# TUI-NICR/nicr-multitask-scene-analysis

Hardware: AMD Instinct MI355X
Metric: Mpix/s panoptic merge+metrics, 640x480xB (higher is better)
Workload: dtype f32; 1 GPU; configs[1]: center-NMS + offset grouping + panoptic merge + mIoU/PQ accumulators (configs[3]); batch_per_gpu=32, global_batch=32, classes=40, height=480, width=640, centers_per_image=24, batches_in_flight=2, parallelism=dp1 (images sharded, accumulators all-reduced once per run, timed)

## Files before the change

nicr_mt_scene_analysis_amd/csrc/panoptic.hip:

```cpp
#include <stdlib.h>
#include <type_traits>

#include "nmsa_common.hpp"
#include "argmax_state.hpp"

namespace nmsa {

constexpr int FUSED_THREADS = 256;
constexpr int FUSED_VOTE_SLOTS = 256;
constexpr int PX_PER_THREAD = 4;
constexpr int PX_PER_ITER = FUSED_THREADS * PX_PER_THREAD;

typedef float f32x4_t __attribute__((ext_vector_type(4)));
typedef unsigned short u16x4_t __attribute__((ext_vector_type(4)));

template <int DTYPE, bool VEC, bool NT = false>
__device__ __forceinline__ float4 load_px4(const void* base, size_t elem_off, int nvalid)
{
    float4 r = make_float4(0.f, 0.f, 0.f, 0.f);
    if (DTYPE == NMSA_F32) {
        const float* p = (const float*)base + elem_off;
        if (VEC && NT) {
            const f32x4_t v = __builtin_nontemporal_load((const f32x4_t*)p);
            return make_float4(v.x, v.y, v.z, v.w);
        }
        if (VEC) return *(const float4*)p;
        if (nvalid > 0) r.x = p[0];
        if (nvalid > 1) r.y = p[1];
        if (nvalid > 2) r.z = p[2];
        if (nvalid > 3) r.w = p[3];
        return r;
    } else {
        const uint16_t* p = (const uint16_t*)base + elem_off;
        uint16_t h[4] = {0, 0, 0, 0};
        if (VEC && NT) {
            const u16x4_t u = __builtin_nontemporal_load((const u16x4_t*)p);
            h[0] = u.x; h[1] = u.y; h[2] = u.z; h[3] = u.w;
        } else if (VEC) {
            const ushort4 u = *(const ushort4*)p;
            h[0] = u.x; h[1] = u.y; h[2] = u.z; h[3] = u.w;
        } else {
            for (int j = 0; j < 4; ++j) if (j < nvalid) h[j] = p[j];
        }
        if (DTYPE == NMSA_BF16) {
            r.x = bf16_to_f32(h[0]); r.y = bf16_to_f32(h[1]);
            r.z = bf16_to_f32(h[2]); r.w = bf16_to_f32(h[3]);
        } else {
            r.x = f16_to_f32(h[0]); r.y = f16_to_f32(h[1]);
            r.z = f16_to_f32(h[2]); r.w = f16_to_f32(h[3]);
        }
        return r;
    }
}

template <int DTYPE>
__device__ __noinline__ int column_class(const void* logits, size_t col0, int P, int C, float m)
{
    auto ld = [&](int c) -> float {
        if (DTYPE == NMSA_F32) return ((const float*)logits)[col0 + (size_t)c * P];
        const uint16_t h = ((const uint16_t*)logits)[col0 + (size_t)c * P];
        return (DTYPE == NMSA_BF16) ? bf16_to_f32(h) : f16_to_f32(h);
    };
    bool nan_or_pinf = false, any_finite = false;
    int first = C, am = C;
    int c = 0;
    for (; c + 4 <= C; c += 4) {
        float v[4];
#pragma unroll
        for (int u = 0; u < 4; ++u) v[u] = ld(c + u);
#pragma unroll
        for (int u = 0; u < 4; ++u) {
            nan_or_pinf |= (v[u] != v[u]) || (v[u] == INFINITY);
            any_finite |= fabsf(v[u]) < INFINITY;
            if (first == C && __fsub_rn(v[u], m) >= TIE_CANDIDATE_GAP) first = c + u;
            if (am == C && v[u] == m) am = c + u;
        }
    }
    for (; c < C; ++c) {
        const float v = ld(c);
        nan_or_pinf |= (v != v) || (v == INFINITY);
        any_finite |= fabsf(v) < INFINITY;
        if (first == C && __fsub_rn(v, m) >= TIE_CANDIDATE_GAP) first = c;
        if (am == C && v == m) am = c;
    }
    if (nan_or_pinf || !any_finite || am == C) return 0;
    if (first >= am) return am;
    return class_by_probability(ld, C, m, am, first, nullptr);
}

template <int DTYPE>
__device__ __noinline__ float2 column_exact(const void* logits, size_t col0, int P, int C)
{
    auto ld = [&](int c) -> float {
        if (DTYPE == NMSA_F32) return ((const float*)logits)[col0 + (size_t)c * P];
        const uint16_t h = ((const uint16_t*)logits)[col0 + (size_t)c * P];
        return (DTYPE == NMSA_BF16) ? bf16_to_f32(h) : f16_to_f32(h);
    };
    bool nan_or_pinf = false, any_finite = false;
    float m = -INFINITY;
    int am = 0;
    for (int c = 0; c < C; ++c) {
        const float v = ld(c);
        if (v != v || v == INFINITY) nan_or_pinf = true;
        if (fabsf(v) < INFINITY) any_finite = true;
        if (v > m) { m = v; am = c; }
    }
    if (nan_or_pinf || !any_finite) return make_float2(__int_as_float(0x7fc00000), __int_as_float(0));
    float se = 0.f;
    int first = am;
    for (int c = 0; c < C; ++c) {
        const float v = ld(c);
        se += (v == -INFINITY) ? 0.f : __expf(v - m);
        if (c < first && __fsub_rn(v, m) >= TIE_CANDIDATE_GAP) first = c;
    }
    if (first >= am) return make_float2(1.0f / se, __int_as_float(am));
    float pm;
    const int cls = class_by_probability(ld, C, m, am, first, &pm);
    return make_float2(pm, __int_as_float(cls));
}

template <bool WITH_SCORE>
__device__ __forceinline__ void argmax_quad(ArgmaxState& st, const float4& a, const float4& b,
                                            const float4& c, const float4& d, int c0,
                                            int nclasses = 4)
{
    if (WITH_SCORE) {
        const float p0[4] = {a.x, b.x, c.x, d.x}, p1[4] = {a.y, b.y, c.y, d.y};
        const float p2[4] = {a.z, b.z, c.z, d.z}, p3[4] = {a.w, b.w, c.w, d.w};
        argmax_group4_score(st, 0, p0, c0);
        argmax_group4_score(st, 1, p1, c0);
        argmax_group4_score(st, 2, p2, c0);
        argmax_group4_score(st, 3, p3, c0);
    } else {
        const float4 q[4] = {a, b, c, d};
#pragma unroll
        for (int u = 0; u < 4; ++u) {
            if (u >= nclasses) break;
            argmax_step<false>(st, 0, q[u].x, c0 + u);
            argmax_step<false>(st, 1, q[u].y, c0 + u);
            argmax_step<false>(st, 2, q[u].z, c0 + u);
            argmax_step<false>(st, 3, q[u].w, c0 + u);
        }
    }
}

__device__ __forceinline__ float sqdist(float cy, float cx, float ly, float lx)
{
    const float dy = __fsub_rn(cy, ly);
    const float dx = __fsub_rn(cx, lx);
    return __fmaf_rn(dx, dx, __fmul_rn(dy, dy));
}

__device__ __forceinline__ float sqrt_tie_upper(float d)
{
    if (!(d < INFINITY)) return d;
    const float dn = __uint_as_float(__float_as_uint(d) + 1u);
    const double m = 0.5 * ((double)d + (double)dn);
    const double m2 = m * m;
    float u = (float)m2;
    if ((double)u >= m2) u = __uint_as_float(__float_as_uint(u) - 1u);
    return u;
}

__device__ __forceinline__ float wave_all_min(float v)
{
#pragma unroll
    for (int o = 32; o > 0; o >>= 1) v = fminf(v, __shfl_xor(v, o));
    return v;
}

struct LdsCenters {
    const float2* cen;
    __device__ __forceinline__ float2 at(int i) const { return cen[i]; }
    __device__ __forceinline__ float2 of_lane(int n) const { return cen[min(lane_id(), n - 1)]; }
};
struct LaneCenters {
    float cy, cx;
    __device__ __forceinline__ float2 at(int i) const
    {
        return make_float2(__int_as_float(__builtin_amdgcn_readlane(__float_as_int(cy), i)),
                           __int_as_float(__builtin_amdgcn_readlane(__float_as_int(cx), i)));
    }
    __device__ __forceinline__ float2 of_lane(int) const { return make_float2(cy, cx); }
};

template <typename Centers>
__device__ __forceinline__ uint64_t wave_candidate_centers(const Centers& cen, int n,
                                                           const float ly[4], const float lx[4],
                                                           const bool act[4])
{
    float lo_y = INFINITY, lo_x = INFINITY, nhi_y = INFINITY, nhi_x = INFINITY;
    bool finite = true;
#pragma unroll
    for (int j = 0; j < 4; ++j) {
        if (act[j]) {
            finite = finite && (fabsf(ly[j]) < INFINITY) && (fabsf(lx[j]) < INFINITY);
            lo_y = fminf(lo_y, ly[j]);  nhi_y = fminf(nhi_y, -ly[j]);
            lo_x = fminf(lo_x, lx[j]);  nhi_x = fminf(nhi_x, -lx[j]);
        }
    }
    const uint64_t all = (n >= 64) ? ~0ull : ((1ull << n) - 1ull);
    if (__any(!finite)) return all;
    lo_y = wave_all_min(lo_y);  nhi_y = wave_all_min(nhi_y);
    lo_x = wave_all_min(lo_x);  nhi_x = wave_all_min(nhi_x);
    if (!(lo_y < INFINITY)) return 0ull;
    const float hi_y = -nhi_y, hi_x = -nhi_x;
    const int lane = lane_id();
    const float2 c = cen.of_lane(n);
    const float a0 = c.x - lo_y, a1 = hi_y - c.x;
    const float b0 = c.y - lo_x, b1 = hi_x - c.y;
    const float near_y = fmaxf(0.f, fmaxf(-a0, -a1)), near_x = fmaxf(0.f, fmaxf(-b0, -b1));
    const float far_y = fmaxf(fabsf(a0), fabsf(a1)), far_x = fmaxf(fabsf(b0), fabsf(b1));
    const float lo = near_y * near_y + near_x * near_x;
    const float hi = (lane < n) ? far_y * far_y + far_x * far_x : INFINITY;
    const float U = wave_all_min(hi);
    return __ballot(lane < n && lo <= U * 1.00001f) & all;
}

template <bool CULL = true, typename Centers = LdsCenters>
__device__ __forceinline__ void group4(const Centers& cen, int n,
                                       const float ly[4], const float lx[4],
                                       const bool act[4], int use_thr, float thr,
                                       uint32_t id[4])
{
    float smin[4], prev[4];
    int imin[4];
    const bool cull = CULL && n <= 64;
    uint64_t m = cull ? wave_candidate_centers(cen, n, ly, lx, act) : 0ull;
    int first = 0;
    if (cull) {
        if (m == 0ull) {
#pragma unroll
            for (int j = 0; j < 4; ++j) id[j] = 0u;
            return;
        }
        first = __ffsll((unsigned long long)m) - 1;
        m &= m - 1;
    }
    {
        const float2 c0 = cen.at(first);
#pragma unroll
        for (int j = 0; j < 4; ++j) {
            smin[j] = sqdist(c0.x, c0.y, ly[j], lx[j]);
            prev[j] = INFINITY;
            imin[j] = first;
        }
    }
    auto visit = [&](const int i) {
        const float2 c = cen.at(i);
#pragma unroll
        for (int j = 0; j < 4; ++j) {
            const float s = sqdist(c.x, c.y, ly[j], lx[j]);
            const bool upd = s < smin[j];
            prev[j] = upd ? smin[j] : prev[j];
            imin[j] = upd ? i : imin[j];
            smin[j] = upd ? s : smin[j];
        }
    };
    if (cull) {
        while (m) {
            const int i = __ffsll((unsigned long long)m) - 1;
            m &= m - 1;
            visit(i);
        }
    } else {
        for (int i = 1; i < n; ++i) visit(i);
    }
    bool maybe_tie = false;
#pragma unroll
    for (int j = 0; j < 4; ++j)
        maybe_tie = maybe_tie || (act[j] && !(prev[j] > fmaf(smin[j], 4.8e-7f, smin[j])));
    int best[4] = {imin[0], imin[1], imin[2], imin[3]};
    if (__any(maybe_tie)) {
        float U[4];
#pragma unroll
        for (int j = 0; j < 4; ++j) U[j] = sqrt_tie_upper(sqrtf(smin[j]));
        for (int i = n - 1; i >= 0; --i) {
            const float2 c = cen.at(i);
#pragma unroll
            for (int j = 0; j < 4; ++j)
                if (sqdist(c.x, c.y, ly[j], lx[j]) <= U[j]) best[j] = i;
        }
#pragma unroll
        for (int j = 0; j < 4; ++j) best[j] = (smin[j] != smin[j]) ? 0 : best[j];
    }
#pragma unroll
    for (int j = 0; j < 4; ++j) {
        uint32_t v = (uint32_t)(best[j] + 1) & 0xFFu;
        if (use_thr && sqrtf(smin[j]) > thr) v = 0;
        id[j] = act[j] ? v : 0u;
    }
}

template <int DTYPE, bool VEC, bool WITH_SCORE, int UNROLL = 8, bool NT = true,
          bool EARLY_OFFSETS = false, bool TILED = false, int TILE_LOG2W = 6>
__global__ __launch_bounds__(FUSED_THREADS) __attribute__((amdgpu_waves_per_eu(5, WITH_SCORE ? 8 : 5))) void k_panoptic_fused(
    const void* __restrict__ logits, const float* __restrict__ offset,
    const int32_t* __restrict__ centers_yx, const int32_t* __restrict__ n_centers,
    const uint8_t* __restrict__ is_thing,
    int C, int H, int W, int max_centers, int iters,
    float scale_y, float scale_x, int use_thr, float thr,
    uint8_t* __restrict__ sem_u8, uint8_t* __restrict__ inst, uint8_t* __restrict__ fg_out,
    float* __restrict__ score, uint32_t* __restrict__ votes, int ablate)
{
    extern __shared__ __align__(16) unsigned char smem[];
    float2* cen = (float2*)smem;
    int* vote_key = (int*)(cen + max_centers);
    uint32_t* vote_cnt = (uint32_t*)(vote_key + FUSED_VOTE_SLOTS);
    const int NC = C + 1;

    const int b = blockIdx.y;
    const int P = H * W;
    const int n = min(n_centers[b], max_centers);

    static_assert(FUSED_THREADS == 256, "one LUT entry per thread");
    static_assert(FUSED_VOTE_SLOTS == FUSED_THREADS, "one vote slot per thread");
    vote_key[threadIdx.x] = -1;
    vote_cnt[threadIdx.x] = 0;
    const bool lane_centers = n <= 64 && H <= 65535 && W <= 65535;
    uint32_t lane_cyx, thing_b = 0u;
    {
        const int2 c2 = *(const int2*)(centers_yx +
            ((size_t)b * max_centers + min(lane_id(), max_centers - 1)) * 2);
        lane_cyx = ((uint32_t)c2.x << 16) | ((uint32_t)c2.y & 0xFFFFu);
#pragma unroll
        for (int k = 0; k < 4; ++k)
            if (k * 64 < C)
                thing_b |= (is_thing[min(k * 64 + lane_id(), C - 1)] != 0 ? 1u : 0u) << k;
    }
    __syncthreads();

    const size_t img_logits = (size_t)b * C * P;
    const float* offy = offset + (size_t)b * 2 * P;
    const float* offx = offy + P;
    uint32_t* votes_b = votes + (size_t)b * 256 * NC;

    const int chunk_start = blockIdx.x * iters * PX_PER_ITER;
    auto chunk = [&](const int it, auto first_tag) {
        constexpr bool FIRST = decltype(first_tag)::value;
        int p0;
        bool active;
        if (TILED) {
            constexpr int TW = 1 << TILE_LOG2W, TH = 1024 >> TILE_LOG2W, LPR = TW / 4;
            const int tiles_x = (W + TW - 1) >> TILE_LOG2W;
            const int tile = blockIdx.x * iters + it;
            const int ty = tile / tiles_x, tx = tile - ty * tiles_x;
            const int row = ty * TH + (int)threadIdx.x / LPR;
            const int col = tx * TW + ((int)threadIdx.x % LPR) * 4;
            active = row < H && col < W;
            p0 = active ? row * W + col : 0;
        } else {
            p0 = chunk_start + it * PX_PER_ITER + threadIdx.x * PX_PER_THREAD;
            active = p0 < P;
        }
        const int nvalid = active ? min(4, P - p0) : 0;

        float4 oy = make_float4(0.f, 0.f, 0.f, 0.f), ox = oy;
        if (EARLY_OFFSETS && active) {
            oy = load_px4<NMSA_F32, VEC, NT>(offy, (size_t)p0, nvalid);
            ox = load_px4<NMSA_F32, VEC, NT>(offx, (size_t)p0, nvalid);
        }


        ArgmaxState st;
        argmax_init(st);
        if (active) {
            int c = 0;
            static_assert(UNROLL % 4 == 0, "class groups of 4");
            for (; c + UNROLL <= C; c += UNROLL) {
                float4 v[UNROLL];
#pragma unroll
                for (int u = 0; u < UNROLL; ++u)
                    v[u] = load_px4<DTYPE, VEC, NT>(logits, img_logits + (size_t)(c + u) * P + p0, nvalid);
#pragma unroll
                for (int u = 0; u < UNROLL; u += 4)
                    argmax_quad<WITH_SCORE>(st, v[u], v[u + 1], v[u + 2], v[u + 3], c + u);
            }
            for (; c < C; c += 4) {
                float4 v[4];
#pragma unroll
                for (int u = 0; u < 4; ++u)
                    v[u] = (c + u < C)
                        ? load_px4<DTYPE, VEC, NT>(logits, img_logits + (size_t)(c + u) * P + p0, nvalid)
                        : make_float4(-INFINITY, -INFINITY, -INFINITY, -INFINITY);
                argmax_quad<WITH_SCORE>(st, v[0], v[1], v[2], v[3], c, min(4, C - c));
            }
        }
        if (FIRST && !lane_centers) {
            for (int i = threadIdx.x; i < n; i += FUSED_THREADS) {
                const int2 c2 = *(const int2*)(centers_yx + ((size_t)b * max_centers + i) * 2);
                cen[i] = make_float2((float)c2.x, (float)c2.y);
            }
            __syncthreads();
        }
        uint64_t thing_m[4];
#pragma unroll
        for (int k = 0; k < 4; ++k)
            thing_m[k] = __ballot(((thing_b >> k) & 1u) != 0u && k * 64 + lane_id() < C);
        int cls[4];
        bool fg[4];
        bool any_fg = false;
#pragma unroll
        for (int j = 0; j < 4; ++j) {
            cls[j] = st.am[j];
            if (WITH_SCORE) {
                float sc = 1.0f / st.se[j];
                if ((st.se[j] != st.se[j] || may_tie_in_probability<DTYPE>(st.m[j])) && j < nvalid) {
                    const float2 ex = column_exact<DTYPE>(logits, img_logits + p0 + j, P, C);
                    sc = ex.x;
                    cls[j] = __float_as_int(ex.y);
                }
                st.se[j] = sc;
            } else if ((st.nf[j] != st.nf[j] || may_tie_in_probability<DTYPE>(st.m[j])) && j < nvalid) {
                cls[j] = column_class<DTYPE>(logits, img_logits + p0 + j, P, C, st.m[j]);
            }
            uint64_t tm = thing_m[0];
            if (C > 64) {
                const int q = cls[j] >> 6;
                tm = (q == 0) ? thing_m[0] : (q == 1) ? thing_m[1] : (q == 2) ? thing_m[2] : thing_m[3];
            }
            fg[j] = (j < nvalid) && ((tm >> (cls[j] & 63)) & 1ull);
            any_fg = any_fg || fg[j];
        }

        uint32_t id[4] = {0u, 0u, 0u, 0u};
        if (__any(any_fg) && n > 0) {
            if (!EARLY_OFFSETS && any_fg && !(ablate & 4)) {
                oy = load_px4<NMSA_F32, VEC, NT>(offy, (size_t)p0, nvalid);
                ox = load_px4<NMSA_F32, VEC, NT>(offx, (size_t)p0, nvalid);
            }
            const float oyv[4] = {oy.x, oy.y, oy.z, oy.w};
            const float oxv[4] = {ox.x, ox.y, ox.z, ox.w};
            float ly[4], lx[4];
            int y = p0 / W, x = p0 - y * W;
#pragma unroll
            for (int j = 0; j < 4; ++j) {
                ly[j] = __fadd_rn((float)y, __fmul_rn(oyv[j], scale_y));
                lx[j] = __fadd_rn((float)x, __fmul_rn(oxv[j], scale_x));
                if (++x == W) { x = 0; ++y; }
            }
            if (ablate & 2) {
#pragma unroll
                for (int j = 0; j < 4; ++j) id[j] = fg[j] ? 1u : 0u;
            } else if (lane_centers) {
                group4(LaneCenters{(float)(lane_cyx >> 16), (float)(lane_cyx & 0xFFFFu)}, n, ly, lx, fg,
                       use_thr, thr, id);
            } else {
                group4(LdsCenters{cen}, n, ly, lx, fg, use_thr, thr, id);
            }
        }

        if (VEC && active) {
            typedef unsigned char u8x4_t __attribute__((ext_vector_type(4)));
            const u8x4_t s4 = {(uint8_t)cls[0], (uint8_t)cls[1], (uint8_t)cls[2], (uint8_t)cls[3]};
            const u8x4_t i4 = {(uint8_t)id[0], (uint8_t)id[1], (uint8_t)id[2], (uint8_t)id[3]};
            const u8x4_t f4 = {(uint8_t)fg[0], (uint8_t)fg[1], (uint8_t)fg[2], (uint8_t)fg[3]};
            if (ablate & 8) {
                __builtin_nontemporal_store(s4, (u8x4_t*)(sem_u8 + (size_t)b * P + p0));
                __builtin_nontemporal_store(i4, (u8x4_t*)(inst + (size_t)b * P + p0));
                if (fg_out) __builtin_nontemporal_store(f4, (u8x4_t*)(fg_out + (size_t)b * P + p0));
            } else {
                *(u8x4_t*)(sem_u8 + (size_t)b * P + p0) = s4;
                *(u8x4_t*)(inst + (size_t)b * P + p0) = i4;
                if (fg_out) *(u8x4_t*)(fg_out + (size_t)b * P + p0) = f4;
            }
            if (WITH_SCORE)
                *(float4*)(score + (size_t)b * P + p0) =
                    make_float4(st.se[0], st.se[1], st.se[2], st.se[3]);
        } else {
            for (int j = 0; j < nvalid; ++j) {
                sem_u8[(size_t)b * P + p0 + j] = (uint8_t)cls[j];
                inst[(size_t)b * P + p0 + j] = (uint8_t)id[j];
                if (fg_out) fg_out[(size_t)b * P + p0 + j] = fg[j];
                if (WITH_SCORE) score[(size_t)b * P + p0 + j] = st.se[j];
            }
        }

        const bool wave_has_inst = __any((id[0] | id[1] | id[2] | id[3]) != 0u);
        if (wave_has_inst && !(ablate & 1)) {
            int key[4];
#pragma unroll
            for (int j = 0; j < 4; ++j)
                key[j] = (id[j] != 0u) ? (int)(id[j] * NC + cls[j] + 1) : -1;
            auto add = [&](int k, uint32_t cnt) {
                const int slot = lds_hash_slot(vote_key, FUSED_VOTE_SLOTS, k);
                if (slot >= 0) atomicAdd(&vote_cnt[slot], cnt);
                else atomicAdd(&votes_b[k], cnt);
            };
            const bool uniform = key[0] == key[1] && key[1] == key[2] && key[2] == key[3];
            int run_len, run_last;
            if (wave_run_head(uniform ? key[0] : -1, run_len, run_last))
                add(key[0], 4u * (uint32_t)run_len);
            if (!uniform) {
#pragma unroll
                for (int j = 0; j < 4; ++j)
                    if (key[j] >= 0) add(key[j], 1u);
            }
        }
    };
    chunk(0, std::true_type{});
    for (int it = 1; it < iters; ++it) chunk(it, std::false_type{});

    __syncthreads();
    {
        const int k = vote_key[threadIdx.x];
        if (k >= 0) atomicAdd(&votes_b[k], vote_cnt[threadIdx.x]);
    }
}

template <int DTYPE, bool VEC, bool WITH_SCORE>
__global__ __launch_bounds__(FUSED_THREADS) void k_semantic_argmax(
    const void* __restrict__ logits, int C, int P,
    uint8_t* __restrict__ idx_u8, int64_t* __restrict__ idx_i64, float* __restrict__ score)
{
    const int b = blockIdx.y;
    const int p0 = (blockIdx.x * FUSED_THREADS + threadIdx.x) * PX_PER_THREAD;
    if (p0 >= P) return;
    const int nvalid = min(4, P - p0);
    const size_t img = (size_t)b * C * P;
    ArgmaxState st;
    argmax_init(st);
    int c = 0;
    for (; c + 8 <= C; c += 8) {
        float4 v[8];
#pragma unroll
        for (int u = 0; u < 8; ++u)
            v[u] = load_px4<DTYPE, VEC, true>(logits, img + (size_t)(c + u) * P + p0, nvalid);
        argmax_quad<WITH_SCORE>(st, v[0], v[1], v[2], v[3], c);
        argmax_quad<WITH_SCORE>(st, v[4], v[5], v[6], v[7], c + 4);
    }
    for (; c < C; c += 4) {
        float4 v[4];
#pragma unroll
        for (int u = 0; u < 4; ++u)
            v[u] = (c + u < C) ? load_px4<DTYPE, VEC, true>(logits, img + (size_t)(c + u) * P + p0, nvalid)
                               : make_float4(-INFINITY, -INFINITY, -INFINITY, -INFINITY);
        argmax_quad<WITH_SCORE>(st, v[0], v[1], v[2], v[3], c, min(4, C - c));
    }
    int cls[4];
    float sc[4];
#pragma unroll
    for (int j = 0; j < 4; ++j) {
        cls[j] = st.am[j];
        sc[j] = 0.f;
        if (WITH_SCORE) {
            sc[j] = 1.0f / st.se[j];
            if ((st.se[j] != st.se[j] || may_tie_in_probability<DTYPE>(st.m[j])) && j < nvalid) {
                const float2 ex = column_exact<DTYPE>(logits, img + p0 + j, P, C);
                sc[j] = ex.x;
                cls[j] = __float_as_int(ex.y);
            }
        } else if ((st.nf[j] != st.nf[j] || may_tie_in_probability<DTYPE>(st.m[j])) && j < nvalid) {
            cls[j] = column_class<DTYPE>(logits, img + p0 + j, P, C, st.m[j]);
        }
    }
    const size_t o = (size_t)b * P + p0;
    if (VEC) {
        if (idx_u8)
            *(uchar4*)(idx_u8 + o) = make_uchar4((uint8_t)cls[0], (uint8_t)cls[1], (uint8_t)cls[2],
                                                 (uint8_t)cls[3]);
        if (idx_i64) {
            *(longlong2*)(idx_i64 + o) = make_longlong2(cls[0], cls[1]);
            *(longlong2*)(idx_i64 + o + 2) = make_longlong2(cls[2], cls[3]);
        }
        if (WITH_SCORE) *(float4*)(score + o) = make_float4(sc[0], sc[1], sc[2], sc[3]);
    } else {
        for (int j = 0; j < nvalid; ++j) {
            if (idx_u8) idx_u8[o + j] = (uint8_t)cls[j];
            if (idx_i64) idx_i64[o + j] = cls[j];
            if (WITH_SCORE) score[o + j] = sc[j];
        }
    }
}

__device__ __forceinline__ float max_nan(float m, float v)
{
    return (v != v) ? v : ((m != m) ? m : fmaxf(m, v));
}

template <int DTYPE>
__device__ __noinline__ void softmax_column_3pass(const void* logits, size_t col0, int P, int C,
                                                  float* probs)
{
    auto ld = [&](int c) -> float {
        if (DTYPE == NMSA_F32) return ((const float*)logits)[col0 + (size_t)c * P];
        const uint16_t h = ((const uint16_t*)logits)[col0 + (size_t)c * P];
        return (DTYPE == NMSA_BF16) ? bf16_to_f32(h) : f16_to_f32(h);
    };
    float m = -INFINITY, sum = 0.f;
    for (int c = 0; c < C; ++c) m = max_nan(m, ld(c));
    for (int c = 0; c < C; ++c) sum += __expf(ld(c) - m);
    for (int c = 0; c < C; ++c) probs[col0 + (size_t)c * P] = __expf(ld(c) - m) / sum;
}

template <int DTYPE, bool VEC>
__global__ __launch_bounds__(FUSED_THREADS) void k_semantic_softmax(
    const void* __restrict__ logits, int C, int P, float* __restrict__ probs)
{
    const int b = blockIdx.y;
    const int p0 = (blockIdx.x * FUSED_THREADS + threadIdx.x) * PX_PER_THREAD;
    if (p0 >= P) return;
    const int nvalid = min(4, P - p0);
    const size_t img = (size_t)b * C * P;
    float m[4] = {-INFINITY, -INFINITY, -INFINITY, -INFINITY};
    float sum[4] = {0.f, 0.f, 0.f, 0.f}, nf[4] = {0.f, 0.f, 0.f, 0.f};
    for (int c = 0; c < C; ++c) {
        const float4 v4 = load_px4<DTYPE, VEC>(logits, img + (size_t)c * P + p0, nvalid);
        const float v[4] = {v4.x, v4.y, v4.z, v4.w};
#pragma unroll
        for (int j = 0; j < 4; ++j) {
            nf[j] = fmaf(v[j], 0.0f, nf[j]);
            const float e = __expf(-fabsf(v[j] - m[j]));
            sum[j] = (v[j] > m[j]) ? fmaf(sum[j], e, 1.0f) : (sum[j] + e);
            m[j] = fmaxf(m[j], v[j]);
        }
    }
    float inv[4];
#pragma unroll
    for (int j = 0; j < 4; ++j) inv[j] = 1.0f / sum[j];
    for (int c = 0; c < C; ++c) {
        const float4 v4 = load_px4<DTYPE, VEC>(logits, img + (size_t)c * P + p0, nvalid);
        const float r[4] = {__expf(v4.x - m[0]) * inv[0], __expf(v4.y - m[1]) * inv[1],
                            __expf(v4.z - m[2]) * inv[2], __expf(v4.w - m[3]) * inv[3]};
        float* o = probs + img + (size_t)c * P + p0;
        if (VEC) {
            f32x4_t q; q.x = r[0]; q.y = r[1]; q.z = r[2]; q.w = r[3];
            __builtin_nontemporal_store(q, (f32x4_t*)o);
        } else {
            for (int j = 0; j < nvalid; ++j) o[j] = r[j];
        }
    }
    for (int j = 0; j < nvalid; ++j)
        if (nf[j] != nf[j]) softmax_column_3pass<DTYPE>(logits, img + p0 + j, P, C, probs);
}

template <int DTYPE, int CMAX>
__global__ __launch_bounds__(FUSED_THREADS) void k_semantic_softmax_reg(
    const void* __restrict__ logits, int C, int P, float* __restrict__ probs)
{
    const int b = blockIdx.y;
    const int p0 = (blockIdx.x * FUSED_THREADS + threadIdx.x) * PX_PER_THREAD;
    if (p0 >= P) return;
    const size_t img = (size_t)b * C * P;
    float4 v[CMAX];
#pragma unroll
    for (int c = 0; c < CMAX; ++c)
        if (c < C) v[c] = load_px4<DTYPE, true, true>(logits, img + (size_t)c * P + p0, 4);
    float m[4] = {-INFINITY, -INFINITY, -INFINITY, -INFINITY};
#pragma unroll
    for (int c = 0; c < CMAX; ++c)
        if (c < C) {
            m[0] = max_nan(m[0], v[c].x); m[1] = max_nan(m[1], v[c].y);
            m[2] = max_nan(m[2], v[c].z); m[3] = max_nan(m[3], v[c].w);
        }
    float sum[4] = {0.f, 0.f, 0.f, 0.f};
#pragma unroll
    for (int c = 0; c < CMAX; ++c)
        if (c < C) {
            v[c].x = __expf(v[c].x - m[0]); v[c].y = __expf(v[c].y - m[1]);
// ... 385 lines not shown

template <bool VEC>
__global__ __launch_bounds__(256) void k_merge_paint(
    const void* __restrict__ sem, int sem_dtype, const void* __restrict__ ins, int ins_dtype,
    const uint8_t* __restrict__ thing_seg, const uint8_t* __restrict__ is_thing_class,
    const int64_t* __restrict__ pan_of_inst, int NC, int P,
    int64_t max_inst, int64_t void_label, int64_t* __restrict__ pan)
{
    __shared__ int64_t s_inst[256];
    const int b = blockIdx.y;
    s_inst[threadIdx.x] = pan_of_inst[(size_t)b * 256 + threadIdx.x];
    __syncthreads();
    for (int p0 = (blockIdx.x * 256 + threadIdx.x) * 4; p0 < P; p0 += gridDim.x * MG_PX_PER_BLOCK) {
        const int nvalid = min(4, P - p0);
        const size_t o = (size_t)b * P + p0;
        int64_t i4[4], s4[4], t4[4], r[4];
        load_int4<VEC>(ins, ins_dtype, o, nvalid, i4);
        load_int4<VEC>(sem, sem_dtype, o, nvalid, s4);
        load_int4<VEC>(thing_seg, NMSA_U8, o, nvalid, t4);
#pragma unroll
        for (int j = 0; j < 4; ++j) {
            r[j] = void_label;
            if (i4[j] != 0) {
                if (i4[j] > 0 && i4[j] < 256 && t4[j]) r[j] = s_inst[i4[j]];
            } else if (s4[j] > 0 && s4[j] < NC && !is_thing_class[s4[j]]) {
                r[j] = s4[j] * max_inst;
            }
        }
        if (VEC) {
            *(longlong2*)(pan + o) = make_longlong2(r[0], r[1]);
            *(longlong2*)(pan + o + 2) = make_longlong2(r[2], r[3]);
        } else {
            for (int j = 0; j < nvalid; ++j) pan[o + j] = r[j];
        }
    }
}

template <bool VEC>
__global__ __launch_bounds__(256) void k_orientation_sums(
    const float* __restrict__ orientation, const uint8_t* __restrict__ inst,
    const uint8_t* __restrict__ mask, int P, double* __restrict__ sums, int32_t* __restrict__ count)
{
    __shared__ double s_sum[256 * 2];
    __shared__ int s_cnt[256];
    const int b = blockIdx.y;
    for (int i = threadIdx.x; i < 512; i += 256) s_sum[i] = 0.0;
    s_cnt[threadIdx.x] = 0;
    __syncthreads();
    const float* o0 = orientation + (size_t)b * 2 * P;
    const float* o1 = o0 + P;
    for (int p0 = (blockIdx.x * 256 + threadIdx.x) * 4; p0 - (int)threadIdx.x * 4 < P;
         p0 += gridDim.x * MG_PX_PER_BLOCK) {
        int id[4] = {0, 0, 0, 0};
        float a[4] = {0.f, 0.f, 0.f, 0.f}, c[4] = {0.f, 0.f, 0.f, 0.f};
        if (p0 < P) {
            const int nvalid = min(4, P - p0);
            const size_t o = (size_t)b * P + p0;
            int64_t i4[4], m4[4] = {1, 1, 1, 1};
            load_int4<VEC>(inst, NMSA_U8, o, nvalid, i4);
            if (mask) load_int4<VEC>(mask, NMSA_U8, o, nvalid, m4);
            if (VEC) {
                const float4 x = *(const float4*)(o0 + p0), y = *(const float4*)(o1 + p0);
                a[0] = x.x; a[1] = x.y; a[2] = x.z; a[3] = x.w;
                c[0] = y.x; c[1] = y.y; c[2] = y.z; c[3] = y.w;
            } else {
                for (int j = 0; j < nvalid; ++j) { a[j] = o0[p0 + j]; c[j] = o1[p0 + j]; }
            }
#pragma unroll
            for (int j = 0; j < 4; ++j) id[j] = (j < nvalid && m4[j]) ? (int)i4[j] : 0;
        }
        const bool same4 = id[0] == id[1] && id[1] == id[2] && id[2] == id[3];
        const int lid = same4 ? id[0] : 0;
        const double l0 = (double)a[0] + (double)a[1] + (double)a[2] + (double)a[3];
        const double l1 = (double)c[0] + (double)c[1] + (double)c[2] + (double)c[3];
        if (lid) {
            atomicAdd(&s_sum[lid * 2 + 0], l0);
            atomicAdd(&s_sum[lid * 2 + 1], l1);
        }
        int run_len, run_last;
        if (wave_run_head(lid ? lid : -1, run_len, run_last)) atomicAdd(&s_cnt[lid], 4 * run_len);
        if (!same4) {
#pragma unroll
            for (int j = 0; j < 4; ++j) {
                if (!id[j]) continue;
                atomicAdd(&s_sum[id[j] * 2 + 0], (double)a[j]);
                atomicAdd(&s_sum[id[j] * 2 + 1], (double)c[j]);
                atomicAdd(&s_cnt[id[j]], 1);
            }
        }
    }
    __syncthreads();
    const int t = threadIdx.x;
    if (s_cnt[t]) {
        atomicAdd(&sums[((size_t)b * 256 + t) * 2 + 0], s_sum[t * 2 + 0]);
        atomicAdd(&sums[((size_t)b * 256 + t) * 2 + 1], s_sum[t * 2 + 1]);
        atomicAdd(&count[(size_t)b * 256 + t], s_cnt[t]);
    }
}

}

using namespace nmsa;

namespace {

int env_int(const char* name, int dflt)
{
    const char* v = getenv(name);
    return v ? atoi(v) : dflt;
}

constexpr int ASSIGN_LDS_WORDS_SMALL = 12 * 1024;
int assign_lds_words(int NC)
{
    int words = ASSIGN_LDS_WORDS;
    if ((size_t)256 * NC * sizeof(uint32_t) > 48 * 1024 &&
        allow_dynamic_lds(k_assign, ASSIGN_LDS_WORDS * sizeof(uint32_t)) != NMSA_OK)
        words = ASSIGN_LDS_WORDS_SMALL;
    return words;
}
size_t assign_lds_bytes(int NC, int words)
{
    int rows = words / NC;
    rows = rows > 256 ? 256 : (rows < 1 ? 1 : rows);
    return (size_t)rows * NC * sizeof(uint32_t);
}

int fused_iters(int P)
{
    (void)P;
    static const int it = env_int("NMSA_FUSED_ITERS", 1);
    return it > 0 ? it : 1;
}

template <int DTYPE>
int launch_fused(const void* logits, const float* offset, const int32_t* centers_yx,
                 const int32_t* n_centers, const uint8_t* is_thing,
                 int B, int C, int H, int W, int max_centers,
                 float sy, float sx, int use_thr, float thr,
                 uint8_t* sem_u8, uint8_t* inst, uint8_t* fg_out, float* score,
                 uint32_t* votes, int vote_rows_hint, hipStream_t stream)
{
    const int P = H * W;
    const int iters = fused_iters(P);
    const int chunks = (P + iters * PX_PER_ITER - 1) / (iters * PX_PER_ITER);
    (void)vote_rows_hint;
    static const int ablate = env_int("NMSA_FUSED_ABLATE", 0);
    const size_t lds = (size_t)max_centers * sizeof(float2) + (size_t)FUSED_VOTE_SLOTS * 8 + 256;
    if (lds > 64 * 1024) return NMSA_ERR_ARG;
    const bool vec = (P % 4 == 0) &&
                     (((uintptr_t)logits | (uintptr_t)offset | (uintptr_t)sem_u8 |
                       (uintptr_t)inst | (uintptr_t)fg_out | (uintptr_t)score) % 16 == 0);
    dim3 grid(chunks, B), block(FUSED_THREADS);
#define NMSA_LAUNCH_FUSED(V, S)                                                              \
    hipLaunchKernelGGL((k_panoptic_fused<DTYPE, V, S>), grid, block, lds, stream, logits,    \
                       offset, centers_yx, n_centers, is_thing, C, H, W, max_centers, iters, \
                       sy, sx, use_thr, thr, sem_u8, inst, fg_out, score, votes, ablate)
    static const int tiled = env_int("NMSA_FUSED_TILED", 2);
    static const int tile_w = env_int("NMSA_FUSED_TILE_W", 128);
    if (vec && !score && W % 4 == 0 && (tiled == 2 || (tiled == 1 && DTYPE != NMSA_F32))) {
        if (tile_w == 64) {
            const int tiles = ((W + 63) / 64) * ((H + 15) / 16);
            hipLaunchKernelGGL((k_panoptic_fused<DTYPE, true, false, 8, true, false, true, 6>),
                               dim3((tiles + iters - 1) / iters, B), block, lds, stream, logits, offset,
                               centers_yx, n_centers, is_thing, C, H, W, max_centers, iters, sy, sx,
                               use_thr, thr, sem_u8, inst, fg_out, score, votes, ablate);
        } else if (tile_w == 256) {
            const int tiles = ((W + 255) / 256) * ((H + 3) / 4);
            hipLaunchKernelGGL((k_panoptic_fused<DTYPE, true, false, 8, true, false, true, 8>),
                               dim3((tiles + iters - 1) / iters, B), block, lds, stream, logits, offset,
                               centers_yx, n_centers, is_thing, C, H, W, max_centers, iters, sy, sx,
                               use_thr, thr, sem_u8, inst, fg_out, score, votes, ablate);
        } else {
            const int tiles = ((W + 127) / 128) * ((H + 7) / 8);
            hipLaunchKernelGGL((k_panoptic_fused<DTYPE, true, false, 8, true, false, true, 7>),
                               dim3((tiles + iters - 1) / iters, B), block, lds, stream, logits, offset,
                               centers_yx, n_centers, is_thing, C, H, W, max_centers, iters, sy, sx,
                               use_thr, thr, sem_u8, inst, fg_out, score, votes, ablate);
        }
    } else if (vec && score && W % 4 == 0 && tiled == 2 && env_int("NMSA_FUSED_SCORE_TILED", 1)) {
        const int tiles = ((W + 127) / 128) * ((H + 7) / 8);
        hipLaunchKernelGGL((k_panoptic_fused<DTYPE, true, true, 8, true, false, true, 7>),
                           dim3((tiles + iters - 1) / iters, B), block, lds, stream, logits, offset,
                           centers_yx, n_centers, is_thing, C, H, W, max_centers, iters, sy, sx,
                           use_thr, thr, sem_u8, inst, fg_out, score, votes, ablate);
    } else if (vec) { if (score) NMSA_LAUNCH_FUSED(true, true); else NMSA_LAUNCH_FUSED(true, false); }
    else { if (score) NMSA_LAUNCH_FUSED(false, true); else NMSA_LAUNCH_FUSED(false, false); }
#undef NMSA_LAUNCH_FUSED
    return check_launch();
}

template <int DTYPE>
int launch_argmax(const void* logits, int B, int C, int P, uint8_t* idx_u8, int64_t* idx_i64,
                  float* score, hipStream_t stream)
{
    const bool vec = (P % 4 == 0) &&
                     (((uintptr_t)logits | (uintptr_t)idx_u8 | (uintptr_t)idx_i64 |
                       (uintptr_t)score) % 16 == 0);
    dim3 grid((P + PX_PER_ITER - 1) / PX_PER_ITER, B), block(FUSED_THREADS);
#define NMSA_LAUNCH_ARGMAX(V, S)                                                          \
    hipLaunchKernelGGL((k_semantic_argmax<DTYPE, V, S>), grid, block, 0, stream, logits,  \
                       C, P, idx_u8, idx_i64, score)
    if (vec) { if (score) NMSA_LAUNCH_ARGMAX(true, true); else NMSA_LAUNCH_ARGMAX(true, false); }
    else { if (score) NMSA_LAUNCH_ARGMAX(false, true); else NMSA_LAUNCH_ARGMAX(false, false); }
#undef NMSA_LAUNCH_ARGMAX
    return check_launch();
}

template <int DTYPE>
int launch_softmax(const void* logits, int B, int C, int P, float* probs, hipStream_t stream)
{
    const bool vec = (P % 4 == 0) && (((uintptr_t)logits | (uintptr_t)probs) % 16 == 0);
    dim3 grid((P + PX_PER_ITER - 1) / PX_PER_ITER, B), block(FUSED_THREADS);
    if (vec && C <= 48 && getenv("NMSA_SOFTMAX_2PASS") == nullptr)
        hipLaunchKernelGGL((k_semantic_softmax_reg<DTYPE, 48>), grid, block, 0, stream, logits, C, P, probs);
    else if (vec) hipLaunchKernelGGL((k_semantic_softmax<DTYPE, true>), grid, block, 0, stream, logits, C, P, probs);
    else hipLaunchKernelGGL((k_semantic_softmax<DTYPE, false>), grid, block, 0, stream, logits, C, P, probs);
    return check_launch();
}

bool bad_dims(int B, int H, int W)
{
    return B <= 0 || H <= 0 || W <= 0 || (int64_t)H * W > ((int64_t)1 << 30) || B > 65535;
}

}

extern "C" int nmsa_group_offsets(const float* offset, const uint8_t* fg,
                                  const int32_t* centers_yx, const int32_t* n_centers,
                                  int B, int H, int W, int max_centers,
                                  float scale_y, float scale_x,
                                  int use_dist_thr, float dist_thr,
                                  uint8_t* inst, int32_t* area, nmsa_stream_t stream_)
{
    hipStream_t stream = (hipStream_t)stream_;
    if (!offset || !fg || !centers_yx || !n_centers || !inst) return NMSA_ERR_ARG;
    if (bad_dims(B, H, W) || max_centers <= 0) return NMSA_ERR_ARG;
    const int P = H * W;
    const size_t lds = (size_t)max_centers * sizeof(float2) + 256 * 4;
    if (lds > 64 * 1024) return NMSA_ERR_ARG;
    int rc;
    if (area) {
        rc = check_hip(hipMemsetAsync(area, 0, (size_t)B * 256 * sizeof(int32_t), stream));
        if (rc) return rc;
    }
    const int iters = 2;
    const int chunks = (P + iters * PX_PER_ITER - 1) / (iters * PX_PER_ITER);
    const bool vec = (P % 4 == 0) &&
                     (((uintptr_t)offset | (uintptr_t)fg | (uintptr_t)inst) % 16 == 0);
    dim3 grid(chunks, B), block(FUSED_THREADS);
    static const int tiled_env = getenv("NMSA_GROUP_TILED") ? atoi(getenv("NMSA_GROUP_TILED")) : 1;
    if (vec && W % 4 == 0 && tiled_env) {
        const int tiles = ((W + 63) / 64) * ((H + 15) / 16);
        hipLaunchKernelGGL((k_group_offsets<true, true>), dim3((tiles + iters - 1) / iters, B), block, lds,
                           stream, offset, fg, centers_yx, n_centers, H, W, max_centers, iters,
                           scale_y, scale_x, use_dist_thr, dist_thr, inst, area);
    } else if (vec)
        hipLaunchKernelGGL(k_group_offsets<true>, grid, block, lds, stream, offset, fg, centers_yx,
                           n_centers, H, W, max_centers, iters, scale_y, scale_x, use_dist_thr,
                           dist_thr, inst, area);
    else
        hipLaunchKernelGGL(k_group_offsets<false>, grid, block, lds, stream, offset, fg, centers_yx,
                           n_centers, H, W, max_centers, iters, scale_y, scale_x, use_dist_thr,
                           dist_thr, inst, area);
    return check_launch();
}

extern "C" int nmsa_semantic_argmax(const void* logits, int logits_dtype,
                                    int B, int C, int H, int W,
                                    uint8_t* idx_u8, int64_t* idx_i64, float* score,
                                    nmsa_stream_t stream_)
{
    hipStream_t stream = (hipStream_t)stream_;
    if (!logits || bad_dims(B, H, W) || C <= 0) return NMSA_ERR_ARG;
    if (idx_u8 && C > 256) return NMSA_ERR_ARG;
    const int P = H * W;
    switch (logits_dtype) {
        case NMSA_F32: return launch_argmax<NMSA_F32>(logits, B, C, P, idx_u8, idx_i64, score, stream);
        case NMSA_BF16: return launch_argmax<NMSA_BF16>(logits, B, C, P, idx_u8, idx_i64, score, stream);
        case NMSA_F16: return launch_argmax<NMSA_F16>(logits, B, C, P, idx_u8, idx_i64, score, stream);
        default: return NMSA_ERR_ARG;
    }
}

extern "C" int nmsa_semantic_softmax(const void* logits, int logits_dtype,
                                     int B, int C, int H, int W, float* probs,
                                     nmsa_stream_t stream_)
{
    hipStream_t stream = (hipStream_t)stream_;
    if (!logits || !probs || bad_dims(B, H, W) || C <= 0) return NMSA_ERR_ARG;
    const int P = H * W;
    switch (logits_dtype) {
        case NMSA_F32: return launch_softmax<NMSA_F32>(logits, B, C, P, probs, stream);
        case NMSA_BF16: return launch_softmax<NMSA_BF16>(logits, B, C, P, probs, stream);
        case NMSA_F16: return launch_softmax<NMSA_F16>(logits, B, C, P, probs, stream);
        default: return NMSA_ERR_ARG;
    }
}

extern "C" int nmsa_panoptic_fused(const void* logits, int logits_dtype, const float* offset,
                                   const int32_t* centers_yx, const int32_t* n_centers,
                                   const uint8_t* is_thing,
                                   int B, int C, int H, int W, int max_centers,
                                   float scale_y, float scale_x,
                                   int use_dist_thr, float dist_thr,
                                   uint8_t* sem_u8, uint8_t* inst, uint8_t* fg_out, float* score,
                                   uint32_t* votes, int votes_are_zero, int vote_rows_hint,
                                   nmsa_stream_t stream_)
{
    hipStream_t stream = (hipStream_t)stream_;
    if (!logits || !offset || !centers_yx || !n_centers || !is_thing || !sem_u8 || !inst || !votes)
        return NMSA_ERR_ARG;
    if (bad_dims(B, H, W) || C <= 0 || C > 256 || max_centers <= 0) return NMSA_ERR_ARG;
    if (!votes_are_zero) {
        int rc = check_hip(hipMemsetAsync(votes, 0, (size_t)B * 256 * (C + 1) * sizeof(uint32_t), stream));
        if (rc) return rc;
    }
    switch (logits_dtype) {
        case NMSA_F32:
            return launch_fused<NMSA_F32>(logits, offset, centers_yx, n_centers, is_thing, B, C, H, W,
                                          max_centers, scale_y, scale_x, use_dist_thr, dist_thr,
                                          sem_u8, inst, fg_out, score, votes, vote_rows_hint, stream);
        case NMSA_BF16:
            return launch_fused<NMSA_BF16>(logits, offset, centers_yx, n_centers, is_thing, B, C, H, W,
                                           max_centers, scale_y, scale_x, use_dist_thr, dist_thr,
                                           sem_u8, inst, fg_out, score, votes, vote_rows_hint, stream);
        case NMSA_F16:
            return launch_fused<NMSA_F16>(logits, offset, centers_yx, n_centers, is_thing, B, C, H, W,
                                          max_centers, scale_y, scale_x, use_dist_thr, dist_thr,
                                          sem_u8, inst, fg_out, score, votes, vote_rows_hint, stream);
        default: return NMSA_ERR_ARG;
    }
}

extern "C" int nmsa_panoptic_assign(uint32_t* votes, int B, int n_vote_classes, int clear_votes,
                                    int64_t max_instances_per_category, int64_t void_label,
                                    int64_t* pan_of_inst, int32_t* area,
                                    int64_t* ids_pan, int64_t* ids_ins, int32_t* n_ids,
                                    nmsa_stream_t stream_)
{
    hipStream_t stream = (hipStream_t)stream_;
// ... 145 lines not shown
```

Baseline: 30730 Mpix/s.

## Restructure fused panoptic kernel codegen: relative plane pointers, inlined rechecks, loop variant

Moves the center staging into LDS ahead of the pixel loop. Logits are now addressed with a per-plane byte pointer plus a 32-bit lane offset, and argmax indices are kept relative to the current class group. The tie/NaN recheck paths are inlined and batched through a bitmask instead of calling noinline functions. A separate LOOP template variant is added for iters>1, using opaque asm barriers to stop the compiler from rematerializing values, and waves-per-EU bounds are made configurable per variant. The goal is lower register pressure and address arithmetic in the hot loop, at the risk of larger code size and different occupancy.

```diff
diff --git a/nicr_mt_scene_analysis_amd/csrc/panoptic.hip b/nicr_mt_scene_analysis_amd/csrc/panoptic.hip
--- a/nicr_mt_scene_analysis_amd/csrc/panoptic.hip
+++ b/nicr_mt_scene_analysis_amd/csrc/panoptic.hip
@@ -7,9 +7,19 @@
 namespace nmsa {
 
 constexpr int FUSED_THREADS = 256;
+#ifndef NMSA_FUSED_WAVES
+#define NMSA_FUSED_WAVES 5
+#endif
+constexpr int fused_waves(bool vec, bool with_score, bool loop)
+{
+    return !vec ? 4 : (with_score || loop) ? 5 : NMSA_FUSED_WAVES;
+}
 constexpr int FUSED_VOTE_SLOTS = 256;
 constexpr int PX_PER_THREAD = 4;
 constexpr int PX_PER_ITER = FUSED_THREADS * PX_PER_THREAD;
+
+__device__ __forceinline__ int opaque_s(int v) { asm volatile("" : "+s"(v)); return v; }
+__device__ __forceinline__ uint32_t opaque_v(uint32_t v) { asm volatile("" : "+v"(v)); return v; }
 
 typedef float f32x4_t __attribute__((ext_vector_type(4)));
 typedef unsigned short u16x4_t __attribute__((ext_vector_type(4)));
@@ -54,7 +64,7 @@
 }
 
 template <int DTYPE>
-__device__ __noinline__ int column_class(const void* logits, size_t col0, int P, int C, float m)
+__device__ __forceinline__ int column_class_body(const void* logits, size_t col0, int P, int C, float m)
 {
     auto ld = [&](int c) -> float {
         if (DTYPE == NMSA_F32) return ((const float*)logits)[col0 + (size_t)c * P];
@@ -87,9 +97,14 @@
     if (first >= am) return am;
     return class_by_probability(ld, C, m, am, first, nullptr);
 }
-
 template <int DTYPE>
-__device__ __noinline__ float2 column_exact(const void* logits, size_t col0, int P, int C)
+__device__ __noinline__ int column_class(const void* logits, size_t col0, int P, int C, float m)
+{
+    return column_class_body<DTYPE>(logits, col0, P, C, m);
+}
+
+template <int DTYPE>
+__device__ __forceinline__ float2 column_exact_body(const void* logits, size_t col0, int P, int C)
 {
     auto ld = [&](int c) -> float {
         if (DTYPE == NMSA_F32) return ((const float*)logits)[col0 + (size_t)c * P];
@@ -118,6 +133,11 @@
     const int cls = class_by_probability(ld, C, m, am, first, &pm);
     return make_float2(pm, __int_as_float(cls));
 }
+template <int DTYPE>
+__device__ __noinline__ float2 column_exact(const void* logits, size_t col0, int P, int C)
+{
+    return column_exact_body<DTYPE>(logits, col0, P, C);
+}
 
 template <bool WITH_SCORE>
 __device__ __forceinline__ void argmax_quad(ArgmaxState& st, const float4& a, const float4& b,
@@ -172,7 +192,12 @@
 struct LdsCenters {
     const float2* cen;
     __device__ __forceinline__ float2 at(int i) const { return cen[i]; }
-    __device__ __forceinline__ float2 of_lane(int n) const { return cen[min(lane_id(), n - 1)]; }
+    __device__ __forceinline__ float2 of_lane(int n) const
+    {
+        int l = lane_id();
+        asm volatile("" : "+v"(l));
+        return cen[min(l, n - 1)];
+    }
 };
 struct LaneCenters {
     float cy, cx;
@@ -293,8 +318,11 @@
 }
 
 template <int DTYPE, bool VEC, bool WITH_SCORE, int UNROLL = 8, bool NT = true,
-          bool EARLY_OFFSETS = false, bool TILED = false, int TILE_LOG2W = 6>
-__global__ __launch_bounds__(FUSED_THREADS) __attribute__((amdgpu_waves_per_eu(5, WITH_SCORE ? 8 : 5))) void k_panoptic_fused(
+          bool EARLY_OFFSETS = false, bool TILED = false, int TILE_LOG2W = 6, bool LOOP = false>
+__global__ __launch_bounds__(FUSED_THREADS)
+__attribute__((amdgpu_waves_per_eu(fused_waves(VEC, WITH_SCORE, LOOP),
+                                   (VEC && !WITH_SCORE && !LOOP) ? NMSA_FUSED_WAVES : 8)))
+void k_panoptic_fused(
     const void* __restrict__ logits, const float* __restrict__ offset,
     const int32_t* __restrict__ centers_yx, const int32_t* __restrict__ n_centers,
     const uint8_t* __restrict__ is_thing,
@@ -328,6 +356,12 @@
             if (k * 64 < C)
                 thing_b |= (is_thing[min(k * 64 + lane_id(), C - 1)] != 0 ? 1u : 0u) << k;
     }
+    if (!lane_centers) {
+        for (int i = threadIdx.x; i < n; i += FUSED_THREADS) {
+            const int2 c2 = *(const int2*)(centers_yx + ((size_t)b * max_centers + i) * 2);
+            cen[i] = make_float2((float)c2.x, (float)c2.y);
+        }
+    }
     __syncthreads();
 
     const size_t img_logits = (size_t)b * C * P;
@@ -336,9 +370,10 @@
     uint32_t* votes_b = votes + (size_t)b * 256 * NC;
 
     const int chunk_start = blockIdx.x * iters * PX_PER_ITER;
-    auto chunk = [&](const int it, auto first_tag) {
-        constexpr bool FIRST = decltype(first_tag)::value;
+    auto chunk = [&](const int it, const int C, const int n, const int ablate, const int use_thr,
+                     const uint32_t thing_b) {
         int p0;
+        int y0 = 0, x0 = 0;
         bool active;
         if (TILED) {
             constexpr int TW = 1 << TILE_LOG2W, TH = 1024 >> TILE_LOG2W, LPR = TW / 4;
@@ -349,6 +384,8 @@
             const int col = tx * TW + ((int)threadIdx.x % LPR) * 4;
             active = row < H && col < W;
             p0 = active ? row * W + col : 0;
+            y0 = row;
+            x0 = col;
         } else {
             p0 = chunk_start + it * PX_PER_ITER + threadIdx.x * PX_PER_THREAD;
             active = p0 < P;
@@ -365,55 +402,72 @@
         ArgmaxState st;
         argmax_init(st);
         if (active) {
+            constexpr size_t ES = (DTYPE == NMSA_F32) ? 4 : 2;
+            const char* plane = (const char*)logits + img_logits * ES;
+            const size_t plane_bytes = (size_t)P * ES;
+            const uint32_t lane_off = (uint32_t)p0 * (uint32_t)ES;
             int c = 0;
             static_assert(UNROLL % 4 == 0, "class groups of 4");
             for (; c + UNROLL <= C; c += UNROLL) {
                 float4 v[UNROLL];
 #pragma unroll
                 for (int u = 0; u < UNROLL; ++u)
-                    v[u] = load_px4<DTYPE, VEC, NT>(logits, img_logits + (size_t)(c + u) * P + p0, nvalid);
+                    v[u] = load_px4<DTYPE, VEC, NT>(plane + (size_t)u * plane_bytes + lane_off, 0, nvalid);
 #pragma unroll
                 for (int u = 0; u < UNROLL; u += 4)
-                    argmax_quad<WITH_SCORE>(st, v[u], v[u + 1], v[u + 2], v[u + 3], c + u);
+                    argmax_quad<WITH_SCORE>(st, v[u], v[u + 1], v[u + 2], v[u + 3], u);
+#pragma unroll
+                for (int j = 0; j < 4; ++j) st.am[j] -= UNROLL;
+                plane += (size_t)UNROLL * plane_bytes;
             }
             for (; c < C; c += 4) {
                 float4 v[4];
 #pragma unroll
                 for (int u = 0; u < 4; ++u)
                     v[u] = (c + u < C)
-                        ? load_px4<DTYPE, VEC, NT>(logits, img_logits + (size_t)(c + u) * P + p0, nvalid)
+                        ? load_px4<DTYPE, VEC, NT>(plane + (size_t)u * plane_bytes + lane_off, 0, nvalid)
                         : make_float4(-INFINITY, -INFINITY, -INFINITY, -INFINITY);
-                argmax_quad<WITH_SCORE>(st, v[0], v[1], v[2], v[3], c, min(4, C - c));
-            }
-        }
-        if (FIRST && !lane_centers) {
-            for (int i = threadIdx.x; i < n; i += FUSED_THREADS) {
-                const int2 c2 = *(const int2*)(centers_yx + ((size_t)b * max_centers + i) * 2);
-                cen[i] = make_float2((float)c2.x, (float)c2.y);
-            }
-            __syncthreads();
+                argmax_quad<WITH_SCORE>(st, v[0], v[1], v[2], v[3], 0, min(4, C - c));
+#pragma unroll
+                for (int j = 0; j < 4; ++j) st.am[j] -= 4;
+                plane += 4 * plane_bytes;
+            }
+#pragma unroll
+            for (int j = 0; j < 4; ++j) st.am[j] += c;
+        }
+        int cls[4];
+        uint32_t recheck = 0u;
+#pragma unroll
+        for (int j = 0; j < 4; ++j) {
+            cls[j] = st.am[j];
+            const float t = WITH_SCORE ? st.se[j] : st.nf[j];
+            if ((t != t || may_tie_in_probability<DTYPE>(st.m[j])) && j < nvalid) recheck |= 1u << j;
+            if (WITH_SCORE) st.se[j] = 1.0f / st.se[j];
+        }
+        while (recheck) {
+            const int j = __ffs(recheck) - 1;
+            recheck &= recheck - 1u;
+            int cj;
+            if (WITH_SCORE) {
+                const float2 ex = column_exact_body<DTYPE>(logits, img_logits + p0 + j, P, C);
+                cj = __float_as_int(ex.y);
+#pragma unroll
+                for (int k = 0; k < 4; ++k) st.se[k] = (k == j) ? ex.x : st.se[k];
+            } else {
+                const float mj = (j == 0) ? st.m[0] : (j == 1) ? st.m[1] : (j == 2) ? st.m[2] : st.m[3];
+                cj = column_class_body<DTYPE>(logits, img_logits + p0 + j, P, C, mj);
+            }
+#pragma unroll
+            for (int k = 0; k < 4; ++k) cls[k] = (k == j) ? cj : cls[k];
         }
         uint64_t thing_m[4];
 #pragma unroll
         for (int k = 0; k < 4; ++k)
             thing_m[k] = __ballot(((thing_b >> k) & 1u) != 0u && k * 64 + lane_id() < C);
-        int cls[4];
         bool fg[4];
         bool any_fg = false;
 #pragma unroll
         for (int j = 0; j < 4; ++j) {
-            cls[j] = st.am[j];
-            if (WITH_SCORE) {
-                float sc = 1.0f / st.se[j];
-                if ((st.se[j] != st.se[j] || may_tie_in_probability<DTYPE>(st.m[j])) && j < nvalid) {
-                    const float2 ex = column_exact<DTYPE>(logits, img_logits + p0 + j, P, C);
-                    sc = ex.x;
-                    cls[j] = __float_as_int(ex.y);
-                }
-                st.se[j] = sc;
-            } else if ((st.nf[j] != st.nf[j] || may_tie_in_probability<DTYPE>(st.m[j])) && j < nvalid) {
-                cls[j] = column_class<DTYPE>(logits, img_logits + p0 + j, P, C, st.m[j]);
-            }
             uint64_t tm = thing_m[0];
             if (C > 64) {
                 const int q = cls[j] >> 6;
@@ -432,7 +486,8 @@
             const float oyv[4] = {oy.x, oy.y, oy.z, oy.w};
             const float oxv[4] = {ox.x, ox.y, ox.z, ox.w};
             float ly[4], lx[4];
-            int y = p0 / W, x = p0 - y * W;
+            int y = y0, x = x0;
+            if (!TILED) { y = p0 / W; x = p0 - y * W; }
 #pragma unroll
             for (int j = 0; j < 4; ++j) {
                 ly[j] = __fadd_rn((float)y, __fmul_rn(oyv[j], scale_y));
@@ -467,12 +522,15 @@
             if (WITH_SCORE)
                 *(float4*)(score + (size_t)b * P + p0) =
                     make_float4(st.se[0], st.se[1], st.se[2], st.se[3]);
-        } else {
-            for (int j = 0; j < nvalid; ++j) {
-                sem_u8[(size_t)b * P + p0 + j] = (uint8_t)cls[j];
-                inst[(size_t)b * P + p0 + j] = (uint8_t)id[j];
-                if (fg_out) fg_out[(size_t)b * P + p0 + j] = fg[j];
-                if (WITH_SCORE) score[(size_t)b * P + p0 + j] = st.se[j];
+        } else if (!VEC) {
+#pragma unroll
+            for (int j = 0; j < 4; ++j) {
+                if (j < nvalid) {
+                    sem_u8[(size_t)b * P + p0 + j] = (uint8_t)cls[j];
+                    inst[(size_t)b * P + p0 + j] = (uint8_t)id[j];
+                    if (fg_out) fg_out[(size_t)b * P + p0 + j] = fg[j];
+                    if (WITH_SCORE) score[(size_t)b * P + p0 + j] = st.se[j];
+                }
             }
         }
 
@@ -498,13 +556,19 @@
             }
         }
     };
-    chunk(0, std::true_type{});
-    for (int it = 1; it < iters; ++it) chunk(it, std::false_type{});
+    if (!LOOP) {
+        chunk(0, C, n, ablate, use_thr, thing_b);
+    } else {
+        for (int it = 0; it < iters; ++it)
+            chunk(it, opaque_s(C), opaque_s(n), opaque_s(ablate), opaque_s(use_thr), opaque_v(thing_b));
+    }
 
     __syncthreads();
     {
-        const int k = vote_key[threadIdx.x];
-        if (k >= 0) atomicAdd(&votes_b[k], vote_cnt[threadIdx.x]);
+        int t = threadIdx.x;
+        asm volatile("" : "+v"(t));
+        const int k = vote_key[t];
+        if (k >= 0) atomicAdd(&votes_b[k], vote_cnt[t]);
     }
 }
 
@@ -1196,41 +1260,39 @@
                      (((uintptr_t)logits | (uintptr_t)offset | (uintptr_t)sem_u8 |
                        (uintptr_t)inst | (uintptr_t)fg_out | (uintptr_t)score) % 16 == 0);
     dim3 grid(chunks, B), block(FUSED_THREADS);
-#define NMSA_LAUNCH_FUSED(V, S)                                                              \
-    hipLaunchKernelGGL((k_panoptic_fused<DTYPE, V, S>), grid, block, lds, stream, logits,    \
-                       offset, centers_yx, n_centers, is_thing, C, H, W, max_centers, iters, \
-                       sy, sx, use_thr, thr, sem_u8, inst, fg_out, score, votes, ablate)
+    using fused_fn = decltype(&k_panoptic_fused<DTYPE, true, false>);
+    fused_fn kernel;
+    const bool loop = iters > 1;
+#define NMSA_FUSED_KERNEL(V, S, T, TW)                                                   \
+    (loop ? (fused_fn)k_panoptic_fused<DTYPE, V, S, 8, true, false, T, TW, true>         \
+          : (fused_fn)k_panoptic_fused<DTYPE, V, S, 8, true, false, T, TW, false>)
     static const int tiled = env_int("NMSA_FUSED_TILED", 2);
     static const int tile_w = env_int("NMSA_FUSED_TILE_W", 128);
+    int tiles = 0;
     if (vec && !score && W % 4 == 0 && (tiled == 2 || (tiled == 1 && DTYPE != NMSA_F32))) {
         if (tile_w == 64) {
-            const int tiles = ((W + 63) / 64) * ((H + 15) / 16);
-            hipLaunchKernelGGL((k_panoptic_fused<DTYPE, true, false, 8, true, false, true, 6>),
-                               dim3((tiles + iters - 1) / iters, B), block, lds, stream, logits, offset,
-                               centers_yx, n_centers, is_thing, C, H, W, max_centers, iters, sy, sx,
-                               use_thr, thr, sem_u8, inst, fg_out, score, votes, ablate);
+            tiles = ((W + 63) / 64) * ((H + 15) / 16);
+            kernel = NMSA_FUSED_KERNEL(true, false, true, 6);
         } else if (tile_w == 256) {
-            const int tiles = ((W + 255) / 256) * ((H + 3) / 4);
-            hipLaunchKernelGGL((k_panoptic_fused<DTYPE, true, false, 8, true, false, true, 8>),
-                               dim3((tiles + iters - 1) / iters, B), block, lds, stream, logits, offset,
-                               centers_yx, n_centers, is_thing, C, H, W, max_centers, iters, sy, sx,
-                               use_thr, thr, sem_u8, inst, fg_out, score, votes, ablate);
+            tiles = ((W + 255) / 256) * ((H + 3) / 4);
+            kernel = NMSA_FUSED_KERNEL(true, false, true, 8);
         } else {
-            const int tiles = ((W + 127) / 128) * ((H + 7) / 8);
-            hipLaunchKernelGGL((k_panoptic_fused<DTYPE, true, false, 8, true, false, true, 7>),
-                               dim3((tiles + iters - 1) / iters, B), block, lds, stream, logits, offset,
-                               centers_yx, n_centers, is_thing, C, H, W, max_centers, iters, sy, sx,
-                               use_thr, thr, sem_u8, inst, fg_out, score, votes, ablate);
+            tiles = ((W + 127) / 128) * ((H + 7) / 8);
+            kernel = NMSA_FUSED_KERNEL(true, false, true, 7);
         }
     } else if (vec && score && W % 4 == 0 && tiled == 2 && env_int("NMSA_FUSED_SCORE_TILED", 1)) {
-        const int tiles = ((W + 127) / 128) * ((H + 7) / 8);
-        hipLaunchKernelGGL((k_panoptic_fused<DTYPE, true, true, 8, true, false, true, 7>),
-                           dim3((tiles + iters - 1) / iters, B), block, lds, stream, logits, offset,
-                           centers_yx, n_centers, is_thing, C, H, W, max_centers, iters, sy, sx,
-                           use_thr, thr, sem_u8, inst, fg_out, score, votes, ablate);
-    } else if (vec) { if (score) NMSA_LAUNCH_FUSED(true, true); else NMSA_LAUNCH_FUSED(true, false); }
-    else { if (score) NMSA_LAUNCH_FUSED(false, true); else NMSA_LAUNCH_FUSED(false, false); }
-#undef NMSA_LAUNCH_FUSED
+        tiles = ((W + 127) / 128) * ((H + 7) / 8);
+        kernel = NMSA_FUSED_KERNEL(true, true, true, 7);
+    } else if (vec) {
+        kernel = score ? NMSA_FUSED_KERNEL(true, true, false, 6) : NMSA_FUSED_KERNEL(true, false, false, 6);
+    } else {
+        kernel = score ? NMSA_FUSED_KERNEL(false, true, false, 6) : NMSA_FUSED_KERNEL(false, false, false, 6);
+    }
+#undef NMSA_FUSED_KERNEL
+    if (tiles > 0) grid = dim3((tiles + iters - 1) / iters, B);
+    hipLaunchKernelGGL(kernel, grid, block, lds, stream, logits, offset, centers_yx, n_centers, is_thing,
+                       C, H, W, max_centers, iters, sy, sx, use_thr, thr, sem_u8, inst, fg_out, score,
+                       votes, ablate);
     return check_launch();
 }
 
```

Result: no change. 30810 Mpix/s, median of 2 (+0.3%).
